# TomClabault/SYCL-ray-tracing

Hardware: AMD Instinct MI355X
Metric: Msamples/sec (W×H×spp/s) at 1080p; per-channel L∞ vs CPU ref (higher is better)
Workload: dtype f32; 1 GPU; cfg2: PBRT Dragon stand-in (1,000,002 tris) 1920x1080x64spp x8 bounces, SKY-L 2048x1024 env IS+MIS; W=1920, H=1080, spp=64, bounces=8, parallelism=1 GPU

## Files before the change

sycl-ray-tracing_amd/csrc/rt_hostsim.cpp:

```cpp
#include <omp.h>

#include <algorithm>
#include <cmath>
#include <cstdlib>
#include <cstring>
#include <vector>

#include "rt_context.h"
#include "rt_denoise.h"
#include "rt_display.h"
#include "rt_query.h"
#include "rt_wave.h"

#ifndef RT_HOSTSIM_SHORT_CAP
#define RT_HOSTSIM_SHORT_CAP 8
#endif
#ifndef RT_HOSTSIM_FAST_CAP
#define RT_HOSTSIM_FAST_CAP 32
#endif
#ifndef RT_HOSTSIM_BUDGET
#define RT_HOSTSIM_BUDGET 24
#endif

int rt_backend_create(rt_context*) { return RT_OK; }
// ... 613 lines not shown
    rtk::heap_order(k, id, m, ok, oi);
    for (int i = 0; i < m; i++) order_emul[i] = oi[i];
    struct QE {
        int id;
        float t;
        bool operator>(const QE& o) const { return t > o.t; }
    };
    std::priority_queue<QE, std::vector<QE>, std::greater<QE>> q;
    for (int i = 0; i < m; i++) q.emplace(QE{i, keys[i]});
    for (int i = 0; i < m; i++) {
        order_std[i] = q.top().id;
        q.pop();
    }
    return 0;
}

#ifndef RT_BUILD_SRC
#define RT_BUILD_SRC "unknown"
#endif
#ifndef RT_BUILD_DEFS
#define RT_BUILD_DEFS ""
#endif
extern "C" const char* rt_build_id(void) { return "src=" RT_BUILD_SRC " defs=" RT_BUILD_DEFS " (hostsim)"; }
```

sycl-ray-tracing_amd/csrc/rt_probe.hip:

```cpp
#include <hip/hip_runtime.h>

#include <algorithm>

#include "rt_backend_hip.h"
#include "rt_wave.h"
#include "rt_wave_layout.h"
#include "rt_quad.h"
#include "rt_row.h"

namespace {

#define RT_LDS_CAP_FAST 16
#define RT_SPILL_FAST RT_FAST_SPILL

template <int N, int M>
struct FastStack {
    static constexpr int CAP = N + M;
    uint32_t* r;
    float* k;
    uint32_t* gr;
    float* gk;
    __device__ __forceinline__ uint32_t rec(int i) const { return i < N ? r[i * 256] : gr[i - N]; }
    __device__ __forceinline__ float key(int i) const { return i < N ? k[i * 256] : gk[i - N]; }
    __device__ __forceinline__ void set(int i, uint32_t rv, float kv)
// ... 70 lines not shown
    const int q = (int)(threadIdx.x >> 2), sub = (int)(threadIdx.x & 3);
    rtk::QuadStack<RT_QSTACK, 64> stk{s_lds + q, (float*)s_lds + RT_QSTACK * 64 + q};
    const int stride = (int)(gridDim.x * blockDim.x) >> 2;
    for (int i = (int)((blockIdx.x * blockDim.x + threadIdx.x) >> 2); i < n; i += stride) {
        rtk::QState qs;
        int res = 1;
        if (rtk::far_origin(S, rtk::v3of(rays[2 * i])))
            res = -1;
        else if (rtk::qstate_begin<ANY>(qs, rtk::v3of(rays[2 * i]), rtk::v3of(rays[2 * i + 1]), sub, nullptr))
            do {
                res = rtk::quad_visit<ANY>(S, qs, stk, sub, nullptr);
            } while (res == 0);
        float t = -1.0f;
        int k = -1;
        const bool ok = res > 0 && (ANY || rtk::quad_closest_answer(S, qs, sub, t, k, nullptr));
        if (sub == 0) {
            if (ANY) {
                out_t[i] = ok ? (float)(qs.h.k == 1 ? 1 : 0) : -2.0f;
                out_k[i] = 0;
            } else {
                out_t[i] = ok ? t : -2.0f;
                out_k[i] = ok ? (k >= 0 ? (int)rt_asuint(S.tri4[3 * (size_t)k].w) : -1) : -2;
            }
        }
    }
}

template <bool ANY>
__global__ __launch_bounds__(256) void k_query_row(RtSceneView S, const float4_* __restrict__ rays,
                                                   float* __restrict__ out_t, int* __restrict__ out_k, int n)
{
    __shared__ uint32_t s_lds[2 * RT_RSTACK * 16];
    const int r = (int)(threadIdx.x >> 4), sub = (int)(threadIdx.x & 15);
    rtk::QuadStack<RT_RSTACK, 16> stk{s_lds + r, (float*)s_lds + RT_RSTACK * 16 + r};
    const int stride = (int)(gridDim.x * blockDim.x) >> 4;
    for (int i = (int)((blockIdx.x * blockDim.x + threadIdx.x) >> 4); i < n; i += stride) {
        rtk::QState qs;
        int res = 1;
        if (rtk::far_origin(S, rtk::v3of(rays[2 * i])))
            res = -1;
        else if (rtk::qstate_begin<ANY>(qs, rtk::v3of(rays[2 * i]), rtk::v3of(rays[2 * i + 1]), sub, nullptr))
            do {
                res = rtk::row_visit<ANY, RT_VISIT_DESCEND>(S, qs, stk, sub, nullptr);
            } while (res == 0);
        float t = -1.0f;
        int k = -1;
// ... 140 lines not shown
            case 2: hipLaunchKernelGGL((k_query<false, 1>), dim3(blocks), dim3(threads), 0, 0, b->view, d_rays, d_t, d_k, n, sr, sk); break;
            case 3: hipLaunchKernelGGL((k_query<true, 1>), dim3(blocks), dim3(threads), 0, 0, b->view, d_rays, d_t, d_k, n, sr, sk); break;
            case 4: hipLaunchKernelGGL((k_query_quad<false, 1>), dim3(qblocks), dim3(threads), 0, 0, b->view, d_rays, d_t, d_k, n); break;
            case 5: hipLaunchKernelGGL((k_query_quad<true, 1>), dim3(qblocks), dim3(threads), 0, 0, b->view, d_rays, d_t, d_k, n); break;
            case 6: hipLaunchKernelGGL((k_query_quad<false, 8>), dim3(qblocks), dim3(threads), 0, 0, b->view, d_rays, d_t, d_k, n); break;
            case 7: hipLaunchKernelGGL((k_query_quad<true, 8>), dim3(qblocks), dim3(threads), 0, 0, b->view, d_rays, d_t, d_k, n); break;
            case 8: hipLaunchKernelGGL((k_query_row<false>), dim3(rblocks), dim3(threads), 0, 0, b->view, d_rays, d_t, d_k, n); break;
            default: hipLaunchKernelGGL((k_query_row<true>), dim3(rblocks), dim3(threads), 0, 0, b->view, d_rays, d_t, d_k, n); break;
        }
    };
    launch();
    HIPCHK(c, hipGetLastError());
    HIPCHK(c, hipEventRecord(b->ev0, 0));
    for (int r = 0; r < reps; r++) launch();
    HIPCHK(c, hipEventRecord(b->ev1, 0));
    HIPCHK(c, hipEventSynchronize(b->ev1));
    float t = 0;
    HIPCHK(c, hipEventElapsedTime(&t, b->ev0, b->ev1));
    if (ms) *ms = t / reps;
    HIPCHK(c, hipMemcpy(out_t, d_t, (size_t)n * 4, hipMemcpyDeviceToHost));
    HIPCHK(c, hipMemcpy(out_k, d_k, (size_t)n * 4, hipMemcpyDeviceToHost));
    return RT_OK;
}
```

sycl-ray-tracing_amd/csrc/rt_quad.h:

```cpp
#pragma once

#include "rt_fast.h"

namespace rtk {

#define RT_QX1 0xB1
#define RT_QX2 0x4E
#define RT_QX3 0x1B

template <int CTRL>
__device__ __forceinline__ int qdpp(int v)
{
    return __builtin_amdgcn_mov_dpp(v, CTRL, 0xF, 0xF, true);
}
template <int CTRL>
__device__ __forceinline__ float qdppf(float v)
{
    return __int_as_float(qdpp<CTRL>(__float_as_int(v)));
}
__device__ __forceinline__ bool s_lower(int sub, int x) { return (sub ^ x) < sub; }
__device__ __forceinline__ int qor(int v)
{
    v |= qdpp<RT_QX1>(v);
    return v | qdpp<RT_QX2>(v);
// ... 30 lines not shown
#define RT_SLAB_QUAD RT_SLABS
#endif

struct QChild {
    int item;
    bool ok;
    float tn;
};
__device__ __forceinline__ QChild quad_child(const RtSceneView& S, int node, int sub, const RayB& rb, float tmax, V3 o,
                                             V3 d)
{
    float4_ a, b;
    child_record(S, node, sub, a, b);
#if RT_SLAB_QUAD
    const float4_ sl = S.bvh4s[4 * (size_t)node + sub];
    rt_pin(sl);
#endif
    rt_pin(a);
    rt_pin(b);
    const int ref = (int)rt_asuint(b.z), cnt = (int)rt_asuint(b.w);
    const float mn[3] = {a.x, a.y, a.z}, mx[3] = {a.w, b.x, b.y};
    QChild c;
    float tf;
    c.ok = cnt >= 0 && box_hit2(mn, mx, rb, tmax, c.tn, tf) && c.tn <= tmax;
#if RT_SLAB_QUAD
    c.ok = c.ok && slab_ok(sl, o, d, c.tn, tf);
#else
    (void)o, (void)d;
#endif
    c.item = cnt > 0 ? leaf_item(ref, cnt) : ref;
    return c;
}

template <bool MARK>
__device__ __forceinline__ float quad_tri(const RtSceneView& S, int item, int sub, V3 o, V3 d, int& k, int& leaf,
                                          int& prim)
{
    const int v = ~item;
    const int first = v >> 2, cnt = (v & 3) + 1;
    float tv = __builtin_inff();
    k = -1;
    leaf = -1;
    prim = 0x7fffffff;
    if (sub < cnt) {
        const float4_* p = S.bvh_tri4 + 3 * (first + sub);
        const float4_ a = p[0], e1 = p[1], e2 = p[2];
        rt_pin(a);
        rt_pin(e1);
        rt_pin(e2);
// ... 96 lines not shown
    q.h.tie = false;
    q.h.ovf = false;
    if (rt_isnan(d.x) || rt_isnan(d.y) || rt_isnan(d.z) || rt_isnan(o.x) || rt_isnan(o.y) || rt_isnan(o.z)) {
        q.h.t = -1.0f;
        return false;
    }
    q.rb = rayb_setup(o, d);
    q.sp = 0;
    q.cur = 0;
    return true;
}

#ifndef RT_VISIT_DESCEND
#define RT_VISIT_DESCEND 2
#endif
#define RT_BRUTE_SCENE (-1)
#define RT_BRUTE_OFF 0
#define RT_BRUTE_ON 1
template <int BRUTE>
__device__ __forceinline__ bool scene_brute(const RtSceneView& S)
{
    return BRUTE == RT_BRUTE_SCENE ? S.brute != 0 : BRUTE == RT_BRUTE_ON;
}
template <bool ANY, int DESC = RT_VISIT_DESCEND, bool PAIR = true, int BRUTE = RT_BRUTE_SCENE, class QSTK>
__device__ __forceinline__ int quad_visit(const RtSceneView& S, QState& q, QSTK& stk, int sub, Stats* st)
{
    FastHit& h = q.h;
    const bool brute = scene_brute<BRUTE>(S);
#pragma unroll 1
    for (int dd = 0; dd < DESC && q.cur >= 0; dd++) {
        if (ANY) {
            constexpr int NW = PAIR ? 2 : 1;
            int nd[NW];
            nd[0] = q.cur;
            int m = 1;
#pragma unroll
            for (int j = 1; j < NW; j++) {
                nd[j] = -1;
                if (m == j && q.sp > 0) {
                    const int t = (int)stk.rec(q.sp - 1);
                    if (t >= 0) {
                        nd[j] = t;
                        q.sp--;
                        m++;
                    }
                }
            }
            if (st && sub == 0) st->c[RT_STAT_ANY_VOL] += 4 * m;
            float4_ r0[NW], r1[NW];
#if RT_SLAB_QUAD
            float4_ sl[NW];
#endif
#pragma unroll
            for (int j = 0; j < NW; j++) {
                r0[j] = r1[j] = float4_{0.0f, 0.0f, 0.0f, 0.0f};
#if RT_SLAB_QUAD
                sl[j] = float4_{0.0f, 0.0f, -__builtin_inff(), __builtin_inff()};
                if (j < m) sl[j] = S.bvh4s[4 * (size_t)nd[j] + sub];
#endif
                if (j < m) child_record(S, nd[j], sub, r0[j], r1[j]);
            }
#pragma unroll
            for (int j = 0; j < NW; j++) {
                rt_pin(r0[j]);
                rt_pin(r1[j]);
#if RT_SLAB_QUAD
                rt_pin(sl[j]);
#endif
            }
            int base = 0, first = 0;
            bool any_first = false;
#pragma unroll
            for (int j = 0; j < NW; j++) {
                const int ref = (int)rt_asuint(r1[j].z), cnt = (int)rt_asuint(r1[j].w);
                const float mn[3] = {r0[j].x, r0[j].y, r0[j].z}, mx[3] = {r0[j].w, r1[j].x, r1[j].y};
                float tn, tf;
#if RT_SLAB_QUAD
                const bool ok = j < m && cnt >= 0 && box_hit2(mn, mx, q.rb, __builtin_inff(), tn, tf) &&
                                slab_ok(sl[j], q.o, q.d, tn, tf);
#else
                const bool ok = j < m && cnt >= 0 && box_hit2(mn, mx, q.rb, __builtin_inff(), tn, tf);
#endif
                const int item = cnt > 0 ? leaf_item(ref, cnt) : ref;
                const int o = ok ? 1 : 0;
                const int o1 = qdpp<RT_QX1>(o), o2 = qdpp<RT_QX2>(o), o3 = qdpp<RT_QX3>(o);
                const int pre = base + (s_lower(sub, 1) ? o1 : 0) + (s_lower(sub, 2) ? o2 : 0) + (s_lower(sub, 3) ? o3 : 0);
                if (ok && pre > 0) {
                    if (q.sp + pre - 1 < QSTK::CAP) stk.set_rec(q.sp + pre - 1, (uint32_t)item);
                }
                if (ok && pre == 0) {
                    first = item;
                    any_first = true;
                }
                base += o + o1 + o2 + o3;
            }
            const int nv = base;
            if (q.sp + nv - 1 > QSTK::CAP) return -1;
            if (nv > 0) {
                q.sp += nv - 1;
                q.cur = qor(any_first ? first : 0);
                continue;
            }
            q.cur = 0x7ffffffe;
            break;
        }
        if (st && sub == 0) st->c[RT_STAT_VOL] += 4;
        const float tmax = h.t + h.t * RT_T2_WINDOW;
        const QChild c = quad_child(S, q.cur, sub, q.rb, tmax, q.o, q.d);
        const float key = c.ok ? c.tn : __builtin_inff();
        const float k1 = qdppf<RT_QX1>(key), k2 = qdppf<RT_QX2>(key), k3 = qdppf<RT_QX3>(key);
        const int s1 = sub ^ 1, s2 = sub ^ 2, s3 = sub ^ 3;
        const int rank = (k1 < key || (k1 == key && s1 < sub) ? 1 : 0) + (k2 < key || (k2 == key && s2 < sub) ? 1 : 0) +
                         (k3 < key || (k3 == key && s3 < sub) ? 1 : 0);
        const int nv = qsum(c.ok ? 1 : 0);
        if (q.sp + nv - 1 > QSTK::CAP) return -1;
        if (c.ok && rank > 0) stk.set(q.sp + nv - 1 - rank, (uint32_t)c.item, key);
        if (nv > 0) {
            q.sp += nv - 1;
            q.cur = qor(c.ok && rank == 0 ? c.item : 0);
            continue;
        }
        q.cur = 0x7ffffffe;
        break;
    }
    if (q.cur >= 0 && q.cur != 0x7ffffffe) return 0;
    if (q.cur < 0) {
        if (st && sub == 0) st->c[ANY ? RT_STAT_ANY_TRI : RT_STAT_TRI] += ((~q.cur) & 3) + 1;
        int k, leaf, prim;
        const float tv = quad_tri<!ANY>(S, q.cur, sub, q.o, q.d, k, leaf, prim);
        if (ANY) {
            const int hitb = tv < __builtin_inff() ? 1 : 0;
            if (brute) {
                if (qor(hitb)) {
                    h.k = 1;
                    return 1;
                }
            } else if (int hm = qor(hitb << sub)) {
                const int l1 = qdpp<RT_QX1>(leaf), l2 = qdpp<RT_QX2>(leaf), l3 = qdpp<RT_QX3>(leaf);
                const ChainRay cr = quad_chain_ray(q.o, q.d, sub);
                int checked = -1;
#pragma unroll 1
                while (hm) {
                    const int x = (__ffs(hm) - 1) ^ sub;
                    hm &= hm - 1;
                    const int lj = x == 0 ? leaf : x == 1 ? l1 : x == 2 ? l2 : l3;
                    if (lj == checked) continue;
                    if (quad_chain_ok(S, cr, lj, false, 0.0f, sub, st)) {
                        h.k = 1;
// ... 21 lines not shown
                h.leaf = wl;
                h.prim = wp;
                h.tie = mixed;
            } else if (m1 == h.t && m1 < __builtin_inff()) {
                h.t2 = __builtin_fminf(h.t2, m2);
                if (brute) {
                    h.tie = true;
                    if (wp < h.prim) h.k = wk, h.leaf = wl, h.prim = wp;
                } else if (!mixed && wl == h.leaf) {
                    if (wk < h.k) h.k = wk, h.prim = wp;
                } else {
                    h.tie = true;
                }
            } else {
                h.t2 = __builtin_fminf(h.t2, m1);
            }
        }
    }
    if (ANY) {
        if (q.sp == 0) return 1;
        q.cur = (int)stk.rec(--q.sp);
        return 0;
    }
    const float tmax = h.t + h.t * RT_T2_WINDOW;
    int nxt = 0x7fffffff;
    while (q.sp > 0) {
        --q.sp;
        const float kk = stk.key(q.sp);
        const int rr = (int)stk.rec(q.sp);
        rt_pin(rr);
        if (kk <= tmax) {
            nxt = rr;
            break;
        }
    }
    q.cur = nxt;
    return nxt == 0x7fffffff ? 1 : 0;
}

template <int BRUTE = RT_BRUTE_SCENE>
__device__ __forceinline__ bool quad_closest_answer(const RtSceneView& S, const QState& q, int sub, float& t_out,
                                                    int& k_out, Stats* st)
{
    const FastHit& h = q.h;
    if (h.k < 0) {
        t_out = -1.0f;
        k_out = -1;
        return true;
    }
    if (RT_FUZZ_CHECK && (h.leaf & RT_FZ_BIT)) return false;
    if (scene_brute<BRUTE>(S)) {
        t_out = h.t;
        k_out = h.k;
        return true;
    }
    if (h.tie) return false;
    const float t2 = __builtin_fminf(h.t2, h.t + h.t * RT_T2_WINDOW);
    if (!quad_chain_ok(S, q.o, q.d, h.leaf, true, t2, sub, st)) return false;
    t_out = h.t;
    k_out = h.k;
// ... 18 lines not shown
```

sycl-ray-tracing_amd/csrc/rt_render.hip:

```cpp
#include <hip/hip_runtime.h>

#include "rt_backend_hip.h"
#include "rt_wave.h"
#include "rt_wave_kernels.h"
#include "rt_quad.h"
#include "rt_row.h"
#include "rt_octet.h"

namespace {

#if RT_DEBUG_FB
__device__ unsigned long long rt_dbg_fb[8];
#define RT_DBG(i) atomicAdd(&rt_dbg_fb[i], 1ull)
#else
#define RT_DBG(i) ((void)0)
#endif
__device__ __forceinline__ int lane_id() { return __lane_id(); }

template <int N>
struct LdsStack {
    static constexpr int CAP = N;
    uint32_t* r;
    float* k;
    __device__ __forceinline__ uint32_t rec(int i) const { return r[i * 256]; }
// ... 415 lines not shown
};

#if RT_DRAIN_STRONG_FENCE
#define RT_DRAIN_FENCE()                                       \
    do {                                                       \
        __builtin_amdgcn_fence(__ATOMIC_SEQ_CST, "workgroup"); \
        __builtin_amdgcn_s_waitcnt(0);                         \
        __builtin_amdgcn_wave_barrier();                       \
    } while (0)
#else
#define RT_DRAIN_FENCE()                                       \
    do {                                                       \
        __builtin_amdgcn_fence(__ATOMIC_ACQ_REL, "wavefront"); \
        __builtin_amdgcn_wave_barrier();                       \
    } while (0)
#endif

template <bool ANY, bool STATS, bool PAIR, int G, int BRUTE, class QSTK>
__device__ __forceinline__ void trace_stream(const rtk::WaveView& W, const RtSceneView& S, QSTK& stk, const int* s_pre,
                                             int first, int total, int wg, int wn, int32_t* fbn, rtk::RayRec* fbl,
                                             rtk::Stats* ps, const QPrefetch& pf)
{
    static_assert(G == 4 || G == 16, "quads or rows");
    constexpr unsigned long long ALL_IDLE = G == 4 ? 0x1111111111111111ull : 0x0001000100010001ull;
    constexpr int REFILL = G == 4 ? RT_TRACE_REFILL : 1;
    const int lane = lane_id(), qd = lane / G;
    int sub = lane & (G - 1);
    int cursor = 0;
    bool exhausted = wg * 16 >= total;
    bool active = false;
    uint32_t target = 0;
    rtk::QState q;
    if (!exhausted) queue_prefetch(W, s_pre, pf, first, cursor, wg, wn, total);
    auto finish = [&](int res, int gs) {
        if (W.r_heavy && sub == 0 && q.calls >= W.heavy_calls) W.r_heavy[target >> 3] = 1;
        if (STATS && W.iterq && sub == 0 && W.iter < RT_MAX_TIMED_ITERS) {
            int32_t* q2 = W.iterq + 2 * RT_MAX_TIMED_ITERS + 4 * W.iter;
            atomicMax(q2 + (ANY ? 1 : 0), q.calls);
            if (q.calls > 8) atomicAdd(q2 + 2, 1);
        }
        float t = 0.0f;
        int k = 0;
        int why = res < 0 ? 3 : 0;
        if (res > 0 && !ANY && !rtk::quad_closest_answer<BRUTE>(S, q, sub & 3, t, k, gs == 4 || sub == 0 ? ps : nullptr)) {
            res = -1;
            why = q.h.tie ? 1 : 2;
        }
        if (STATS && W.wlog && sub == 0 && q.calls >= W.wlog_min)
            walk_log(W, q.o, q.d, target, q.calls, res <= 0 ? -2.0f : ANY ? (float)(q.h.k == 1) : t, res <= 0 ? why : k,
                     gs == 4 ? 0 : 1);
        if (sub == 0) {
            if (res > 0) {
                if (ANY)
                    rtk::finish_any(W, target, q.h.k == 1);
                else
                    rtk::finish_closest(W, target, q.o, q.d, t, k);
            } else {
                fbl[atomicAdd(fbn, 1)] = rtk::RayRec{rtk::f4(q.o, rt_asfloat(target >> 3)),
                                                     rtk::f4(q.d, rt_asfloat(target & 7u))};
                RT_DBG(ANY ? 2 : 0);
                RT_DBG(why == 3 ? 3 : why == 1 ? 4 : 5);
                if (gs == 16) RT_DBG(6);
                atomicAdd(&W.r_park[target >> 3], 1);
                if (STATS && W.iterq && W.iter < RT_MAX_TIMED_ITERS)
                    atomicAdd(W.iterq + 2 * RT_MAX_TIMED_ITERS + 4 * W.iter + 3, 1);
            }
        }
    };
    for (;;) {
        const unsigned long long bidle = __ballot(!active && sub == 0);
        if (!exhausted && (__popcll(bidle) >= REFILL || bidle == ALL_IDLE)) {
            if (!active) {
                const int j = cursor + __popcll(bidle & ((1ull << (qd * G)) - 1ull));
                const int idx = (wg + (j >> 4) * wn) * 16 + (j & 15);
                if (idx < total) {
                    const int slot = j - cursor;
                    __builtin_amdgcn_s_waitcnt(0x0F70);
                    rtk::RayRec r;
                    r.o = pf.buf[2 * slot];
                    r.d = pf.buf[2 * slot + 1];
                    const int kind = pf.kind[slot];
                    target = (rt_asuint(r.o.w) << 3) | (uint32_t)kind;
                    if (forced_fallback(W, r.o, r.d)) {
                        if (sub == 0) {
                            r.d.w = rt_asfloat(target & 7u);
                            fbl[atomicAdd(fbn, 1)] = r;
                            atomicAdd(&W.r_park[target >> 3], 1);
                        }
                    } else if (rtk::qstate_begin<ANY>(q, rtk::v3of(r.o), rtk::v3of(r.d), sub, ps)) {
                        active = true;
                        q.calls = 0;
                    } else if (sub == 0) {
                        if (ANY)
                            rtk::finish_any(W, target, false);
                        else
                            rtk::finish_closest(W, target, q.o, q.d, -1.0f, -1);
                    }
                }
            }
            cursor += __popcll(bidle);
            exhausted = (wg + (cursor >> 4) * wn) * 16 >= total;
            __builtin_amdgcn_fence(__ATOMIC_ACQ_REL, "wavefront");
            __builtin_amdgcn_wave_barrier();
            if (!exhausted) queue_prefetch(W, s_pre, pf, first, cursor, wg, wn, total);
            if (STATS && lane == 0) ps->c[RT_STAT_REFILLS]++;
        }
        const unsigned long long bact = __ballot(active && sub == 0);
        if (!bact) {
            if (exhausted) break;
            continue;
        }
        if (G == 4 && W.drain_rows > 0 && exhausted && __popcll(bact) <= W.drain_rows) break;
        if (STATS) {
            if (active && sub == 0) ps->c[exhausted ? RT_STAT_DRAIN_VISITS : RT_STAT_QUAD_VISITS]++;
            if (lane == 0) ps->c[exhausted ? RT_STAT_DRAIN_SLOTS : RT_STAT_WAVE_SLOTS] += 64 / G;
        }
        if (active) {
            int res;
            if constexpr (G == 4)
                res = rtk::quad_visit<ANY, RT_VISIT_DESCEND, PAIR, BRUTE>(S, q, stk, sub, ps);
            else
                res = rtk::row_visit<ANY, RT_VISIT_DESCEND, BRUTE>(S, q, stk, sub, ps);
            q.calls += G == 4 ? 1 : 2;
            if (res != 0) {
                active = false;
                finish(res, G);
            }
        }
    }
    if constexpr (G == 4) {
        const unsigned long long bact = __ballot(active && sub == 0);
        if (!bact) return;
        const int row = lane >> 4;
        unsigned long long m = bact;
        for (int i = 0; i < row; i++) m &= m - 1ull;
// ... 9 lines not shown
        for (int i = 0; i < 3; i++) q.rb.inv[i] = pf(q.rb.inv[i]), q.rb.oi[i] = pf(q.rb.oi[i]);
        q.h.t = pf(q.h.t), q.h.t2 = pf(q.h.t2), q.h.k = pi(q.h.k), q.h.leaf = pi(q.h.leaf);
        if (BRUTE != RT_BRUTE_OFF) q.h.prim = pi(q.h.prim);
        q.h.tie = pi(q.h.tie ? 1 : 0) != 0;
        q.sp = pi(q.sp), q.cur = pi(q.cur), q.calls = pi(q.calls);
        target = (uint32_t)pi((int)target);
        sub = lane & 15;
        const int wq = (int)(threadIdx.x >> 6) * 16;
        uint32_t* qr = stk.r - (threadIdx.x >> 2) + wq;
        float* qk = stk.k - (threadIdx.x >> 2) + wq;
        const int sq = src >> 2;
        uint32_t r0 = 0, r1 = 0;
        float k0 = 0.0f, k1 = 0.0f;
        if (ract && sub < q.sp) r0 = qr[sub * 64 + sq], k0 = qk[sub * 64 + sq];
        if (ract && sub + 16 < q.sp) r1 = qr[(sub + 16) * 64 + sq], k1 = qk[(sub + 16) * 64 + sq];
        RT_DRAIN_FENCE();
        RowInQuadStack rs{qr + 4 * row, qk + 4 * row};
        if (ract && sub < q.sp) rs.set(sub, r0, k0);
        if (ract && sub + 16 < q.sp) rs.set(sub + 16, r1, k1);
        RT_DRAIN_FENCE();
        active = ract;
#if RT_DRAIN_RESTART == 1
        q.sp = 0;
        if (q.cur != 0x7fffffff) q.cur = 0;
#elif RT_DRAIN_RESTART == 2
        if (ract) rtk::qstate_begin<ANY>(q, q.o, q.d, sub, nullptr);
#elif RT_DRAIN_RESTART == 3
        q.rb = rtk::rayb_setup(q.o, q.d);
#elif RT_DRAIN_RESTART == 4
        q.h.t = __builtin_inff(), q.h.t2 = __builtin_inff(), q.h.k = ANY ? 0 : -1, q.h.leaf = -1;
        q.h.prim = 0x7fffffff, q.h.tie = false, q.h.ovf = false;
        q.sp = 0;
        if (q.cur != 0x7fffffff) q.cur = 0;
#endif
        while (__any(active)) {
            if (STATS) {
                if (active && sub == 0) ps->c[RT_STAT_DRAIN_VISITS]++;
                if (lane == 0) ps->c[RT_STAT_DRAIN_SLOTS] += 4;
            }
            if (active) {
                const int res = rtk::row_visit<ANY, RT_VISIT_DESCEND, BRUTE>(S, q, rs, sub, ps);
                q.calls += 2;
                if (res != 0) {
                    active = false;
                    finish(res, 16);
                }
            }
        }
    }
}

template <bool STATS, bool PAIR = true, int G = 4, int BRUTE = RT_BRUTE_SCENE>
__global__ __launch_bounds__(256) __attribute__((amdgpu_waves_per_eu(RT_TRACE_OCC, 8))) void k_trace(rtk::WaveView W, int par, unsigned long long* stats)
{
    __shared__ uint32_t s_lds[RT_LDS_WORDS * 256];
    __shared__ int s_pre[RT_NSEG + 1];
// ... 352 lines not shown
```

sycl-ray-tracing_amd/csrc/rt_row.h:

```cpp
#pragma once

#include "rt_quad.h"

namespace rtk {

#ifndef RT_SLAB_ROW
#define RT_SLAB_ROW RT_SLABS
#endif

#define RT_DPP_ROW_MIRROR 0x140
#define RT_DPP_ROW_HALF_MIRROR 0x141
#define RT_DPP_ROW_ROR(k) (0x120 + (k))

template <int CTRL>
__device__ __forceinline__ int rdpp(int v)
{
    return __builtin_amdgcn_mov_dpp(v, CTRL, 0xF, 0xF, true);
}
template <int CTRL>
__device__ __forceinline__ float rdppf(float v)
{
    return __int_as_float(rdpp<CTRL>(__float_as_int(v)));
}
__device__ __forceinline__ int row_or(int v)
// ... 18 lines not shown
    return __builtin_fminf(v, rdppf<RT_DPP_ROW_MIRROR>(v));
}
template <int K>
__device__ __forceinline__ int row_rank_from(float key, int sub)
{
    const float o = rdppf<RT_DPP_ROW_ROR(K)>(key);
    const int os = rdpp<RT_DPP_ROW_ROR(K)>(sub);
    const int c = (o < key || (o == key && os < sub)) ? 1 : 0;
    if constexpr (K < 15)
        return c + row_rank_from<K + 1>(key, sub);
    else
        return c;
}
__device__ __forceinline__ int row_rank(float key, int sub) { return row_rank_from<1>(key, sub); }

__device__ __forceinline__ unsigned row_bits(unsigned long long b) { return (unsigned)(b >> (__lane_id() & 48)) & 0xFFFFu; }

template <bool ANY, int DESC, int BRUTE = RT_BRUTE_SCENE, class RSTK>
__device__ __forceinline__ int row_visit(const RtSceneView& S, QState& q, RSTK& stk, int sub, Stats* st)
{
    FastHit& h = q.h;
    const bool brute = scene_brute<BRUTE>(S);
#pragma unroll 1
    for (int dd = 0; dd < DESC && q.cur >= 0; dd++) {
        const float4_* p = (const float4_*)(S.bvh16 + (size_t)q.cur * RT_BVH16_W + sub);
        const float4_ a = p[0], b = p[1];
#if RT_SLAB_ROW
        const float4_ sl = S.bvh16s[(size_t)q.cur * RT_BVH16_W + sub];
        rt_pin(sl);
#endif
        rt_pin(a);
        rt_pin(b);
        const int ref = (int)rt_asuint(b.z), cnt = (int)rt_asuint(b.w);
        const float mn[3] = {a.x, a.y, a.z}, mx[3] = {a.w, b.x, b.y};
        const float tmax = ANY ? __builtin_inff() : h.t + h.t * RT_T2_WINDOW;
        float tn, tf;
#if RT_SLAB_ROW
        const bool ok = cnt >= 0 && box_hit2(mn, mx, q.rb, tmax, tn, tf) && (ANY || tn <= tmax) && slab_ok(sl, q.o, q.d, tn, tf);
#else
        const bool ok = cnt >= 0 && box_hit2(mn, mx, q.rb, tmax, tn, tf) && (ANY || tn <= tmax);
#endif
        const int item = cnt > 0 ? leaf_item(ref, cnt) : ref;
        const unsigned m = row_bits(__ballot(ok));
        const int nv = __popc(m);
        if (st) {
            const int nb = __popc(row_bits(__ballot(cnt >= 0)));
            if (sub == 0) st->c[ANY ? RT_STAT_ANY_VOL : RT_STAT_VOL] += nb;
        }
        if (q.sp + nv - 1 > RSTK::CAP) return -1;
        int first;
        if (ANY) {
            const int pre = __popc(m & ((1u << sub) - 1u));
            if (ok && pre > 0) stk.set_rec(q.sp + pre - 1, (uint32_t)item);
            first = ok && pre == 0;
        } else {
            const float key = ok ? __builtin_fminf(tn, 3.0e38f) : __builtin_inff();
            const int rank = row_rank(key, sub);
            if (ok && rank > 0) stk.set(q.sp + nv - 1 - rank, (uint32_t)item, key);
            first = ok && rank == 0;
        }
        if (nv > 0) {
            q.sp += nv - 1;
            q.cur = row_or(first ? item : 0);
            continue;
        }
        q.cur = 0x7ffffffe;
        break;
    }
    if (q.cur >= 0 && q.cur != 0x7ffffffe) return 0;
    if (q.cur < 0) {
        int l0 = q.cur, l1 = 0, l2 = 0, l3 = 0, nl = 1;
        const float tw = h.t + h.t * RT_T2_WINDOW;
#pragma unroll
        for (int g = 1; g < 4; g++) {
            if (nl != g || q.sp == 0) break;
            const int t = (int)stk.rec(q.sp - 1);
            const float tk = ANY ? 0.0f : stk.key(q.sp - 1);
            if (!ANY) rt_pin(tk);
            if (t >= 0 || (!ANY && !(tk <= tw))) break;
            q.sp--;
            nl++;
            (g == 1 ? l1 : g == 2 ? l2 : l3) = t;
        }
        if (st && sub == 0) {
            int nt = ((~l0) & 3) + 1;
            if (nl > 1) nt += ((~l1) & 3) + 1;
            if (nl > 2) nt += ((~l2) & 3) + 1;
            if (nl > 3) nt += ((~l3) & 3) + 1;
            st->c[ANY ? RT_STAT_ANY_TRI : RT_STAT_TRI] += nt;
        }
        const int g = sub >> 2;
        const int mine_leaf = g == 0 ? l0 : g == 1 ? l1 : g == 2 ? l2 : l3;
// ... 36 lines not shown
                h.leaf = wl;
                h.prim = wp;
                h.tie = mixed;
            } else if (m1 == h.t && m1 < __builtin_inff()) {
                h.t2 = __builtin_fminf(h.t2, m2);
                if (brute) {
                    h.tie = true;
                    if (wp < h.prim) h.k = wk, h.leaf = wl, h.prim = wp;
                } else if (!mixed && wl == h.leaf) {
                    if (wk < h.k) h.k = wk, h.prim = wp;
                } else {
                    h.tie = true;
                }
            } else {
                h.t2 = __builtin_fminf(h.t2, m1);
            }
        }
    }
    if (ANY) {
        if (q.sp == 0) return 1;
        q.cur = (int)stk.rec(--q.sp);
        return 0;
    }
    const float tmax = h.t + h.t * RT_T2_WINDOW;
    int nxt = 0x7fffffff;
    while (q.sp > 0) {
        --q.sp;
        const float kk = stk.key(q.sp);
        const int rr = (int)stk.rec(q.sp);
        rt_pin(rr);
        if (kk <= tmax) {
            nxt = rr;
            break;
        }
    }
    q.cur = nxt;
    return nxt == 0x7fffffff ? 1 : 0;
}

}
```

sycl-ray-tracing_amd/rt_amd/_capi.py:

```python
from __future__ import annotations

import ctypes
import os

PKG_DIR = os.path.dirname(os.path.dirname(os.path.abspath(__file__)))
LIB_DIR = os.path.join(PKG_DIR, "lib")
PRODUCT = os.environ.get("RT_HIP_LIB") or os.path.join(LIB_DIR, "librt_hip.so")
HOSTSIM = os.environ.get("RT_HOSTSIM_LIB") or os.path.join(LIB_DIR, "librt_hostsim.so")

EXPORTS = [
    "rt_create", "rt_destroy", "rt_last_error", "rt_version", "rt_build_id", "rt_set_scene", "rt_build_bvh",
    "rt_set_bvh_preorder", "rt_bvh_dump", "rt_bvh_info", "rt_set_env", "rt_set_camera", "rt_render",
    "rt_render_device", "rt_render_pixels", "rt_intersect", "rt_set_stats", "rt_get_stats", "rt_last_kernel_ms",
    "rt_mesh_load", "rt_mesh_counts", "rt_mesh_copy", "rt_mesh_free", "rt_camera_preset", "rt_env_luminance_cdf",
    "rt_octree_dump", "rt_read_hdr", "rt_write_png", "rt_image_to_rgba8",
    "rt_set_intersect_mode", "rt_create_multi", "rt_device_count", "rt_set_materials", "rt_render_variants",
    "rt_create_multi_loopback", "rt_test_create_multi_rccl", "rt_test_fail_device", "rt_test_schedule", "rt_test_walk_log",
    "rt_test_walk_log_read", "rt_test_obj_parallel_min", "rt_device_env_search",
    "rt_camera_rays", "rt_render_features", "rt_render_features_device", "rt_denoise_default_params", "rt_denoise",
    "rt_denoise_device",
    "rt_query", "rt_query_device", "rt_query_last_exact",
    "rt_progress_begin", "rt_progress_advance", "rt_progress_resolve", "rt_progress_resolve_device",
    "rt_progress_info", "rt_progress_save", "rt_progress_load", "rt_progress_end",
    "rt_display_default_params", "rt_render_linear", "rt_render_linear_device", "rt_progress_resolve_linear",
# ... 72 lines not shown
    "rt_progress_begin": (I, [P, I, I, I, I, P, I, I]),
    "rt_progress_advance": (I, [P, I, P]),
    "rt_progress_resolve": (I, [P, P]),
    "rt_progress_resolve_device": (I, [P, P, P]),
    "rt_progress_info": (I, [P, P]),
    "rt_progress_save": (L, [P, P, L]),
    "rt_progress_load": (I, [P, P, L]),
    "rt_progress_end": (None, [P]),
    "rt_display_default_params": (None, [ctypes.POINTER(DisplayParams)]),
    "rt_render_linear": (I, [P, I, I, I, I, P]),
    "rt_render_linear_device": (I, [P, I, I, I, I, P, I, I, P]),
    "rt_progress_resolve_linear": (I, [P, P]),
    "rt_progress_resolve_linear_device": (I, [P, P, P]),
    "rt_display": (I, [P, I, I, P, ctypes.POINTER(DisplayParams), P, P]),
    "rt_display_device": (I, [P, I, I, P, ctypes.POINTER(DisplayParams), P, P, P]),
    "rt_write_hdr": (I, [ctypes.c_char_p, P, I, I, I]),
    "rt_device_libm": (I, [I, I, P, P, P, I]),
    "rt_device_last_kernel_ms": (ctypes.c_double, [P]),
    "rt_device_kernel_timing": (I, [P, I, P, P]),
    "rt_device_set_lanes": (I, [P, I]),
    "rt_device_last_iterations": (I, [P]),
    "rt_device_exact_handovers": (I, [P, P, I]),
    "rt_device_queries": (I, [P, I, P, I, I, P, P, P]),
    "rt_device_denoise_pass_ms": (I, [P, I, P, I]),
    "rt_device_display_kernel_ms": (I, [P, I, I, P, P, P, P, I, P]),
    "rt_hostsim_heap_order": (I, [P, I, P, P]),
    "rt_hostsim_fast_queries": (I, [P, P, I, P, P]),
    "rt_hostsim_leaf_hits": (I, [P, P, I, P]),
}

QUERY_CLOSEST, QUERY_ANY, QUERY_EXACT = 0, 1, 0x100

STAT_NAMES = ["rays", "vol", "tri", "leaf", "mat", "env", "cdf", "heap_slow", "any_rays", "any_vol", "any_tri",
              "any_leaf", "verify", "fallback", "quad_visits", "wave_slots", "refills", "drain_slots", "drain_visits",
              "steps"]

_libs: dict = {}


class RtError(RuntimeError):
    pass


def lib(hostsim: bool = False):
    path = HOSTSIM if hostsim else PRODUCT
    if path in _libs:
        return _libs[path]
    if not os.path.exists(path):
        raise RtError(f"{path} is not built: run `make` (or __graft_entry__.build()) first")
    L_ = ctypes.CDLL(path)
    for name, (res, args) in _SIGS.items():
# ... 19 lines not shown
```

Before: 1094 Msamples/s.

## Make quad BVH visit branch-free and unify refill trigger in trace loop

Rewrites the quad traversal step with bitwise predicates and select operations in place of early returns and branches. It introduces sentinel cursor states (overflow, pop, none) and a shared pop_within helper that replaces the duplicated pop loops. The wave scheduling loop now uses a single precomputed refill threshold, which also folds the drain condition into that check. The goal is to cut divergence and scalar branch overhead in the hot traversal loop. It also adds diagnostic trip-count kernels on host and device, and the heavier predicated work may add ALU cost or change drain behaviour.

```diff
diff --git a/sycl-ray-tracing_amd/csrc/rt_hostsim.cpp b/sycl-ray-tracing_amd/csrc/rt_hostsim.cpp
--- a/sycl-ray-tracing_amd/csrc/rt_hostsim.cpp
+++ b/sycl-ray-tracing_amd/csrc/rt_hostsim.cpp
@@ -659,3 +659,86 @@
 #define RT_BUILD_DEFS ""
 #endif
 extern "C" const char* rt_build_id(void) { return "src=" RT_BUILD_SRC " defs=" RT_BUILD_DEFS " (hostsim)"; }
+
+extern "C" int rt_hostsim_trip_cases(rt_context* c, const float* rays, int n, int* out)
+{
+    if (!c || n < 0 || (n > 0 && (!rays || !out))) return RT_ERR_ARG;
+    if (!c->have_bvh) return RT_ERR_STATE;
+    const RtSceneView S = rt_host_view(c);
+#pragma omp parallel
+    {
+        rtk::IdxStack<RT_HOSTSIM_FAST_CAP> stk;
+#pragma omp for schedule(dynamic, 64)
+        for (int i = 0; i < n; i++) {
+            const float* r = rays + 6 * (size_t)i;
+            const rtk::V3 o = rtk::v3(r[0], r[1], r[2]), d = rtk::v3(r[3], r[4], r[5]);
+            int* w = out + 10 * (size_t)i;
+            for (int j = 0; j < 10; j++) w[j] = 0;
+            if (rt_isnan(o.x) || rt_isnan(o.y) || rt_isnan(o.z) || rt_isnan(d.x) || rt_isnan(d.y) || rt_isnan(d.z)) continue;
+            rtk::FastHit h;
+            h.t = h.t2 = __builtin_inff();
+            h.k = -1, h.leaf = -1, h.prim = 0x7fffffff, h.tie = false, h.ovf = false;
+            const rtk::RayB rb = rtk::rayb_setup(o, d);
+            int sp = 0, cur = 0;
+            for (;;) {
+                rtk::ItemRecs R;
+                rtk::load_item(S, cur, R);
+                if (cur >= 0) {
+                    const rtk::Bvh4R nd = rtk::node_of(R);
+                    float tn[4], kk[4];
+                    bool hit[4];
+                    int v[4], ix[4] = {0, 1, 2, 3}, nv = 0;
+                    const float tmax = h.t + h.t * RT_T2_WINDOW;
+                    rtk::box4(S, cur, nd, rb, o, d, tmax, tn, hit);
+                    for (int ch = 0; ch < 4; ch++) {
+                        const bool ok = hit[ch] && tn[ch] <= tmax;
+                        kk[ch] = ok ? tn[ch] : __builtin_inff();
+                        v[ch] = nd.cnt[ch] > 0 ? rtk::leaf_item(nd.ref[ch], nd.cnt[ch]) : nd.ref[ch];
+                        nv += ok ? 1 : 0;
+                    }
+                    rtk::sort4(kk, ix);
+                    w[nv]++;
+                    for (int j = 1; j < nv; j++)
+                        if (kk[j] == kk[j - 1]) {
+                            w[5]++;
+                            break;
+                        }
+                    if (sp + nv - 1 > RT_HOSTSIM_FAST_CAP) {
+                        w[6] = sp + nv - 1;
+                        w[8] = 1;
+                        break;
+                    }
+                    for (int j = nv - 1; j >= 1; j--) stk.set(sp++, (uint32_t)v[ix[j]], kk[j]);
+                    if (sp > w[6]) w[6] = sp;
+                    if (nv > 0) {
+                        cur = v[ix[0]];
+                        continue;
+                    }
+                } else {
+                    const int cnt = ((~cur) & 3) + 1;
+                    w[9]++;
+                    for (int j = 0; j < cnt; j++) {
+                        float t;
+                        if (rtk::tri_test_v(rtk::ld3(R.q[3 * j]), rtk::ld3(R.q[3 * j + 1]), rtk::ld3(R.q[3 * j + 2]), o, d, t))
+                            rtk::fast_take(h, t, (int)rt_asuint(R.q[3 * j].w), (int)rt_asuint(R.q[3 * j + 1].w),
+                                           (int)rt_asuint(R.q[3 * j + 2].w), S.brute != 0);
+                    }
+                }
+                const float tmax = h.t + h.t * RT_T2_WINDOW;
+                cur = 0x7fffffff;
+                while (sp > 0) {
+                    --sp;
+                    if (stk.key(sp) <= tmax) {
+                        cur = (int)stk.rec(sp);
+                        break;
+                    }
+                }
+                if (cur == 0x7fffffff) {
+                    w[7]++;
+                    break;
+                }
+            }
+        }
+    }
+    return RT_OK;
+}
diff --git a/sycl-ray-tracing_amd/csrc/rt_probe.hip b/sycl-ray-tracing_amd/csrc/rt_probe.hip
--- a/sycl-ray-tracing_amd/csrc/rt_probe.hip
+++ b/sycl-ray-tracing_amd/csrc/rt_probe.hip
@@ -116,6 +116,32 @@
                 out_t[i] = ok ? t : -2.0f;
                 out_k[i] = ok ? (k >= 0 ? (int)rt_asuint(S.tri4[3 * (size_t)k].w) : -1) : -2;
             }
+        }
+    }
+}
+
+template <bool ANY>
+__global__ __launch_bounds__(256) void k_query_quad_trips(RtSceneView S, const float4_* __restrict__ rays, int* __restrict__ out, int n)
+{
+    __shared__ uint32_t s_lds[2 * RT_QSTACK * 64];
+    const int q = (int)(threadIdx.x >> 2), sub = (int)(threadIdx.x & 3);
+    rtk::QuadStack<RT_QSTACK, 64> stk{s_lds + q, (float*)s_lds + RT_QSTACK * 64 + q};
+    const int stride = (int)(gridDim.x * blockDim.x) >> 2;
+    for (int i = (int)((blockIdx.x * blockDim.x + threadIdx.x) >> 2); i < n; i += stride) {
+        rtk::QState qs;
+        rtk::Stats st;
+        for (int j = 0; j < RT_STAT_COUNT; j++) st.c[j] = 0;
+        int calls = 0, res = 1;
+        if (!rtk::far_origin(S, rtk::v3of(rays[2 * i])) &&
+            rtk::qstate_begin<ANY>(qs, rtk::v3of(rays[2 * i]), rtk::v3of(rays[2 * i + 1]), sub, &st))
+            do {
+                res = rtk::quad_visit<ANY>(S, qs, stk, sub, &st);
+                calls++;
+            } while (res == 0);
+        if (sub == 0) {
+            out[3 * i] = calls;
+            out[3 * i + 1] = (int)st.c[ANY ? RT_STAT_ANY_VOL : RT_STAT_VOL];
+            out[3 * i + 2] = (int)st.c[ANY ? RT_STAT_ANY_TRI : RT_STAT_TRI];
         }
     }
 }
@@ -302,3 +328,27 @@
     HIPCHK(c, hipMemcpy(out_k, d_k, (size_t)n * 4, hipMemcpyDeviceToHost));
     return RT_OK;
 }
+
+extern "C" int rt_device_query_trips(rt_context* c, int any, const float* rays, int n, int* out)
+{
+    if (!c || !c->backend || n <= 0 || !rays || !out || (any != 0 && any != 1)) return RT_ERR_ARG;
+    Backend* b = rt_backend_dev0(c);
+    HIPCHK(c, hipSetDevice(b->device));
+    if (c->dirty) {
+        if (int r = rt_backend_upload(c)) return r;
+        c->dirty = false;
+    }
+    const int threads = 256, qblocks = std::min((4 * n + threads - 1) / threads, 4096);
+    DevBuf b_rays, b_out;
+    if (int r = ensure(c, b_rays, (size_t)n * 32)) return r;
+    if (int r = ensure(c, b_out, (size_t)n * 12)) return r;
+    HIPCHK(c, hipMemcpy(b_rays.p, rays, (size_t)n * 32, hipMemcpyHostToDevice));
+    if (any)
+        hipLaunchKernelGGL((k_query_quad_trips<true>), dim3(qblocks), dim3(threads), 0, 0, b->view, (const float4_*)b_rays.p, (int*)b_out.p, n);
+    else
+        hipLaunchKernelGGL((k_query_quad_trips<false>), dim3(qblocks), dim3(threads), 0, 0, b->view, (const float4_*)b_rays.p, (int*)b_out.p, n);
+    HIPCHK(c, hipGetLastError());
+    HIPCHK(c, hipDeviceSynchronize());
+    HIPCHK(c, hipMemcpy(out, b_out.p, (size_t)n * 12, hipMemcpyDeviceToHost));
+    return RT_OK;
+}
diff --git a/sycl-ray-tracing_amd/csrc/rt_quad.h b/sycl-ray-tracing_amd/csrc/rt_quad.h
--- a/sycl-ray-tracing_amd/csrc/rt_quad.h
+++ b/sycl-ray-tracing_amd/csrc/rt_quad.h
@@ -76,9 +76,10 @@
     const float mn[3] = {a.x, a.y, a.z}, mx[3] = {a.w, b.x, b.y};
     QChild c;
     float tf;
-    c.ok = cnt >= 0 && box_hit2(mn, mx, rb, tmax, c.tn, tf) && c.tn <= tmax;
-#if RT_SLAB_QUAD
-    c.ok = c.ok && slab_ok(sl, o, d, c.tn, tf);
+    const bool box = box_hit2(mn, mx, rb, tmax, c.tn, tf);
+    c.ok = (cnt >= 0) & box & (c.tn <= tmax);
+#if RT_SLAB_QUAD
+    c.ok = c.ok & slab_ok(sl, o, d, c.tn, tf);
 #else
     (void)o, (void)d;
 #endif
@@ -221,13 +222,37 @@
 {
     return BRUTE == RT_BRUTE_SCENE ? S.brute != 0 : BRUTE == RT_BRUTE_ON;
 }
+constexpr int RT_CUR_OVF = 0x7ffffffd;
+constexpr int RT_CUR_POP = 0x7ffffffe;
+constexpr int RT_CUR_NONE = 0x7fffffff;
+__device__ __forceinline__ bool cur_inner(int cur) { return (unsigned)cur < (unsigned)RT_CUR_OVF; }
+
+template <class STK>
+__device__ __forceinline__ int pop_within(const STK& stk, int& sp, float tmax)
+{
+    int nxt = RT_CUR_NONE;
+    bool more;
+    do {
+        const bool has = sp > 0;
+        const int d = has ? sp - 1 : 0;
+        const float kk = stk.key(d);
+        const int rr = (int)stk.rec(d);
+        rt_pin(rr);
+        const bool take = has & (kk <= tmax);
+        nxt = take ? rr : nxt;
+        sp = d;
+        more = has & !take;
+    } while (more);
+    return nxt;
+}
+
 template <bool ANY, int DESC = RT_VISIT_DESCEND, bool PAIR = true, int BRUTE = RT_BRUTE_SCENE, class QSTK>
 __device__ __forceinline__ int quad_visit(const RtSceneView& S, QState& q, QSTK& stk, int sub, Stats* st)
 {
     FastHit& h = q.h;
     const bool brute = scene_brute<BRUTE>(S);
 #pragma unroll 1
-    for (int dd = 0; dd < DESC && q.cur >= 0; dd++) {
+    for (int dd = 0; dd < DESC && cur_inner(q.cur); dd++) {
         if (ANY) {
             constexpr int NW = PAIR ? 2 : 1;
             int nd[NW];
@@ -235,15 +260,11 @@
             int m = 1;
 #pragma unroll
             for (int j = 1; j < NW; j++) {
-                nd[j] = -1;
-                if (m == j && q.sp > 0) {
-                    const int t = (int)stk.rec(q.sp - 1);
-                    if (t >= 0) {
-                        nd[j] = t;
-                        q.sp--;
-                        m++;
-                    }
-                }
+                const int t = (int)stk.rec(q.sp > 0 ? q.sp - 1 : 0);
+                const bool tk = (m == j) & (q.sp > 0) & (t >= 0);
+                nd[j] = tk ? t : -1;
+                q.sp -= tk ? 1 : 0;
+                m += tk ? 1 : 0;
             }
             if (st && sub == 0) st->c[RT_STAT_ANY_VOL] += 4 * m;
             float4_ r0[NW], r1[NW];
@@ -268,40 +289,29 @@
 #endif
             }
             int base = 0, first = 0;
-            bool any_first = false;
 #pragma unroll
             for (int j = 0; j < NW; j++) {
                 const int ref = (int)rt_asuint(r1[j].z), cnt = (int)rt_asuint(r1[j].w);
                 const float mn[3] = {r0[j].x, r0[j].y, r0[j].z}, mx[3] = {r0[j].w, r1[j].x, r1[j].y};
                 float tn, tf;
-#if RT_SLAB_QUAD
-                const bool ok = j < m && cnt >= 0 && box_hit2(mn, mx, q.rb, __builtin_inff(), tn, tf) &&
-                                slab_ok(sl[j], q.o, q.d, tn, tf);
-#else
-                const bool ok = j < m && cnt >= 0 && box_hit2(mn, mx, q.rb, __builtin_inff(), tn, tf);
+                bool ok = (j < m) & (cnt >= 0) & box_hit2(mn, mx, q.rb, __builtin_inff(), tn, tf);
+#if RT_SLAB_QUAD
+                ok = ok & slab_ok(sl[j], q.o, q.d, tn, tf);
 #endif
                 const int item = cnt > 0 ? leaf_item(ref, cnt) : ref;
                 const int o = ok ? 1 : 0;
                 const int o1 = qdpp<RT_QX1>(o), o2 = qdpp<RT_QX2>(o), o3 = qdpp<RT_QX3>(o);
                 const int pre = base + (s_lower(sub, 1) ? o1 : 0) + (s_lower(sub, 2) ? o2 : 0) + (s_lower(sub, 3) ? o3 : 0);
-                if (ok && pre > 0) {
-                    if (q.sp + pre - 1 < QSTK::CAP) stk.set_rec(q.sp + pre - 1, (uint32_t)item);
-                }
-                if (ok && pre == 0) {
-                    first = item;
-                    any_first = true;
-                }
+                if (ok & (pre > 0) & (q.sp + pre - 1 < QSTK::CAP)) stk.set_rec(q.sp + pre - 1, (uint32_t)item);
+                first |= (ok & (pre == 0)) ? item : 0;
                 base += o + o1 + o2 + o3;
             }
             const int nv = base;
-            if (q.sp + nv - 1 > QSTK::CAP) return -1;
-            if (nv > 0) {
-                q.sp += nv - 1;
-                q.cur = qor(any_first ? first : 0);
-                continue;
-            }
-            q.cur = 0x7ffffffe;
-            break;
+            const bool ovf = q.sp + nv - 1 > QSTK::CAP;
+            const int nxt = qor(first);
+            q.sp += ((nv > 0) & !ovf) ? nv - 1 : 0;
+            q.cur = ovf ? RT_CUR_OVF : nv > 0 ? nxt : RT_CUR_POP;
+            continue;
         }
         if (st && sub == 0) st->c[RT_STAT_VOL] += 4;
         const float tmax = h.t + h.t * RT_T2_WINDOW;
@@ -312,17 +322,14 @@
         const int rank = (k1 < key || (k1 == key && s1 < sub) ? 1 : 0) + (k2 < key || (k2 == key && s2 < sub) ? 1 : 0) +
                          (k3 < key || (k3 == key && s3 < sub) ? 1 : 0);
         const int nv = qsum(c.ok ? 1 : 0);
-        if (q.sp + nv - 1 > QSTK::CAP) return -1;
-        if (c.ok && rank > 0) stk.set(q.sp + nv - 1 - rank, (uint32_t)c.item, key);
-        if (nv > 0) {
-            q.sp += nv - 1;
-            q.cur = qor(c.ok && rank == 0 ? c.item : 0);
-            continue;
-        }
-        q.cur = 0x7ffffffe;
-        break;
-    }
-    if (q.cur >= 0 && q.cur != 0x7ffffffe) return 0;
+        const bool ovf = q.sp + nv - 1 > QSTK::CAP;
+        if (c.ok & (rank > 0) & !ovf) stk.set(q.sp + nv - 1 - rank, (uint32_t)c.item, key);
+        const int nxt = qor((c.ok & (rank == 0)) ? c.item : 0);
+        q.sp += ((nv > 0) & !ovf) ? nv - 1 : 0;
+        q.cur = ovf ? RT_CUR_OVF : nv > 0 ? nxt : RT_CUR_POP;
+    }
+    if (cur_inner(q.cur)) return 0;
+    if (q.cur == RT_CUR_OVF) return -1;
     if (q.cur < 0) {
         if (st && sub == 0) st->c[ANY ? RT_STAT_ANY_TRI : RT_STAT_TRI] += ((~q.cur) & 3) + 1;
         int k, leaf, prim;
@@ -390,20 +397,8 @@
         q.cur = (int)stk.rec(--q.sp);
         return 0;
     }
-    const float tmax = h.t + h.t * RT_T2_WINDOW;
-    int nxt = 0x7fffffff;
-    while (q.sp > 0) {
-        --q.sp;
-        const float kk = stk.key(q.sp);
-        const int rr = (int)stk.rec(q.sp);
-        rt_pin(rr);
-        if (kk <= tmax) {
-            nxt = rr;
-            break;
-        }
-    }
-    q.cur = nxt;
-    return nxt == 0x7fffffff ? 1 : 0;
+    q.cur = pop_within(stk, q.sp, h.t + h.t * RT_T2_WINDOW);
+    return q.cur == RT_CUR_NONE ? 1 : 0;
 }
 
 template <int BRUTE = RT_BRUTE_SCENE>
diff --git a/sycl-ray-tracing_amd/csrc/rt_render.hip b/sycl-ray-tracing_amd/csrc/rt_render.hip
--- a/sycl-ray-tracing_amd/csrc/rt_render.hip
+++ b/sycl-ray-tracing_amd/csrc/rt_render.hip
@@ -461,7 +461,6 @@
                                              rtk::Stats* ps, const QPrefetch& pf)
 {
     static_assert(G == 4 || G == 16, "quads or rows");
-    constexpr unsigned long long ALL_IDLE = G == 4 ? 0x1111111111111111ull : 0x0001000100010001ull;
     constexpr int REFILL = G == 4 ? RT_TRACE_REFILL : 1;
     const int lane = lane_id(), qd = lane / G;
     int sub = lane & (G - 1);
@@ -506,50 +505,57 @@
             }
         }
     };
+    constexpr int NGROUPS = 64 / G;
+    static_assert(REFILL <= NGROUPS, "all groups idle triggers a refill");
+    const int trig_done = NGROUPS - (G == 4 && W.drain_rows > 0 ? min(W.drain_rows, NGROUPS) : 0);
+    int trig = exhausted ? trig_done : REFILL;
     for (;;) {
         const unsigned long long bidle = __ballot(!active && sub == 0);
-        if (!exhausted && (__popcll(bidle) >= REFILL || bidle == ALL_IDLE)) {
-            if (!active) {
-                const int j = cursor + __popcll(bidle & ((1ull << (qd * G)) - 1ull));
-                const int idx = (wg + (j >> 4) * wn) * 16 + (j & 15);
-                if (idx < total) {
-                    const int slot = j - cursor;
-                    __builtin_amdgcn_s_waitcnt(0x0F70);
-                    rtk::RayRec r;
-                    r.o = pf.buf[2 * slot];
-                    r.d = pf.buf[2 * slot + 1];
-                    const int kind = pf.kind[slot];
-                    target = (rt_asuint(r.o.w) << 3) | (uint32_t)kind;
-                    if (forced_fallback(W, r.o, r.d)) {
-                        if (sub == 0) {
-                            r.d.w = rt_asfloat(target & 7u);
-                            fbl[atomicAdd(fbn, 1)] = r;
-                            atomicAdd(&W.r_park[target >> 3], 1);
+        if (__popcll(bidle) >= trig) {
+            if (!exhausted) {
+                if (!active) {
+                    const int j = cursor + __popcll(bidle & ((1ull << (qd * G)) - 1ull));
+                    const int idx = (wg + (j >> 4) * wn) * 16 + (j & 15);
+                    if (idx < total) {
+                        const int slot = j - cursor;
+                        __builtin_amdgcn_s_waitcnt(0x0F70);
+                        rtk::RayRec r;
+                        r.o = pf.buf[2 * slot];
+                        r.d = pf.buf[2 * slot + 1];
+                        const int kind = pf.kind[slot];
+                        target = (rt_asuint(r.o.w) << 3) | (uint32_t)kind;
+                        if (forced_fallback(W, r.o, r.d)) {
+                            if (sub == 0) {
+                                r.d.w = rt_asfloat(target & 7u);
+                                fbl[atomicAdd(fbn, 1)] = r;
+                                atomicAdd(&W.r_park[target >> 3], 1);
+                            }
+                        } else if (rtk::qstate_begin<ANY>(q, rtk::v3of(r.o), rtk::v3of(r.d), sub, ps)) {
+                            active = true;
+                            q.calls = 0;
+                        } else if (sub == 0) {
+                            if (ANY)
+                                rtk::finish_any(W, target, false);
+                            else
+                                rtk::finish_closest(W, target, q.o, q.d, -1.0f, -1);
                         }
-                    } else if (rtk::qstate_begin<ANY>(q, rtk::v3of(r.o), rtk::v3of(r.d), sub, ps)) {
-                        active = true;
-                        q.calls = 0;
-                    } else if (sub == 0) {
-                        if (ANY)
-                            rtk::finish_any(W, target, false);
-                        else
-                            rtk::finish_closest(W, target, q.o, q.d, -1.0f, -1);
                     }
                 }
-            }
-            cursor += __popcll(bidle);
-            exhausted = (wg + (cursor >> 4) * wn) * 16 >= total;
-            __builtin_amdgcn_fence(__ATOMIC_ACQ_REL, "wavefront");
-            __builtin_amdgcn_wave_barrier();
-            if (!exhausted) queue_prefetch(W, s_pre, pf, first, cursor, wg, wn, total);
-            if (STATS && lane == 0) ps->c[RT_STAT_REFILLS]++;
-        }
-        const unsigned long long bact = __ballot(active && sub == 0);
-        if (!bact) {
-            if (exhausted) break;
-            continue;
-        }
-        if (G == 4 && W.drain_rows > 0 && exhausted && __popcll(bact) <= W.drain_rows) break;
+                cursor += __popcll(bidle);
+                exhausted = (wg + (cursor >> 4) * wn) * 16 >= total;
+                __builtin_amdgcn_fence(__ATOMIC_ACQ_REL, "wavefront");
+                __builtin_amdgcn_wave_barrier();
+                if (!exhausted) queue_prefetch(W, s_pre, pf, first, cursor, wg, wn, total);
+                if (STATS && lane == 0) ps->c[RT_STAT_REFILLS]++;
+                trig = exhausted ? trig_done : REFILL;
+            }
+            const unsigned long long bact = __ballot(active && sub == 0);
+            if (!bact) {
+                if (exhausted) break;
+                continue;
+            }
+            if (G == 4 && W.drain_rows > 0 && exhausted && __popcll(bact) <= W.drain_rows) break;
+        }
         if (STATS) {
             if (active && sub == 0) ps->c[exhausted ? RT_STAT_DRAIN_VISITS : RT_STAT_QUAD_VISITS]++;
             if (lane == 0) ps->c[exhausted ? RT_STAT_DRAIN_SLOTS : RT_STAT_WAVE_SLOTS] += 64 / G;
@@ -605,7 +611,7 @@
         active = ract;
 #if RT_DRAIN_RESTART == 1
         q.sp = 0;
-        if (q.cur != 0x7fffffff) q.cur = 0;
+        if (q.cur != rtk::RT_CUR_NONE) q.cur = 0;
 #elif RT_DRAIN_RESTART == 2
         if (ract) rtk::qstate_begin<ANY>(q, q.o, q.d, sub, nullptr);
 #elif RT_DRAIN_RESTART == 3
@@ -614,7 +620,7 @@
         q.h.t = __builtin_inff(), q.h.t2 = __builtin_inff(), q.h.k = ANY ? 0 : -1, q.h.leaf = -1;
         q.h.prim = 0x7fffffff, q.h.tie = false, q.h.ovf = false;
         q.sp = 0;
-        if (q.cur != 0x7fffffff) q.cur = 0;
+        if (q.cur != rtk::RT_CUR_NONE) q.cur = 0;
 #endif
         while (__any(active)) {
             if (STATS) {
diff --git a/sycl-ray-tracing_amd/csrc/rt_row.h b/sycl-ray-tracing_amd/csrc/rt_row.h
--- a/sycl-ray-tracing_amd/csrc/rt_row.h
+++ b/sycl-ray-tracing_amd/csrc/rt_row.h
@@ -64,7 +64,7 @@
     FastHit& h = q.h;
     const bool brute = scene_brute<BRUTE>(S);
 #pragma unroll 1
-    for (int dd = 0; dd < DESC && q.cur >= 0; dd++) {
+    for (int dd = 0; dd < DESC && cur_inner(q.cur); dd++) {
         const float4_* p = (const float4_*)(S.bvh16 + (size_t)q.cur * RT_BVH16_W + sub);
         const float4_ a = p[0], b = p[1];
 #if RT_SLAB_ROW
@@ -106,10 +106,10 @@
             q.cur = row_or(first ? item : 0);
             continue;
         }
-        q.cur = 0x7ffffffe;
+        q.cur = RT_CUR_POP;
         break;
     }
-    if (q.cur >= 0 && q.cur != 0x7ffffffe) return 0;
+    if (cur_inner(q.cur)) return 0;
     if (q.cur < 0) {
         int l0 = q.cur, l1 = 0, l2 = 0, l3 = 0, nl = 1;
         const float tw = h.t + h.t * RT_T2_WINDOW;
@@ -192,20 +192,8 @@
         q.cur = (int)stk.rec(--q.sp);
         return 0;
     }
-    const float tmax = h.t + h.t * RT_T2_WINDOW;
-    int nxt = 0x7fffffff;
-    while (q.sp > 0) {
-        --q.sp;
-        const float kk = stk.key(q.sp);
-        const int rr = (int)stk.rec(q.sp);
-        rt_pin(rr);
-        if (kk <= tmax) {
-            nxt = rr;
-            break;
-        }
-    }
-    q.cur = nxt;
-    return nxt == 0x7fffffff ? 1 : 0;
+    q.cur = pop_within(stk, q.sp, h.t + h.t * RT_T2_WINDOW);
+    return q.cur == RT_CUR_NONE ? 1 : 0;
 }
 
 }
diff --git a/sycl-ray-tracing_amd/rt_amd/_capi.py b/sycl-ray-tracing_amd/rt_amd/_capi.py
--- a/sycl-ray-tracing_amd/rt_amd/_capi.py
+++ b/sycl-ray-tracing_amd/rt_amd/_capi.py
@@ -118,11 +118,13 @@
     "rt_device_last_iterations": (I, [P]),
     "rt_device_exact_handovers": (I, [P, P, I]),
     "rt_device_queries": (I, [P, I, P, I, I, P, P, P]),
+    "rt_device_query_trips": (I, [P, I, P, I, P]),
     "rt_device_denoise_pass_ms": (I, [P, I, P, I]),
     "rt_device_display_kernel_ms": (I, [P, I, I, P, P, P, P, I, P]),
     "rt_hostsim_heap_order": (I, [P, I, P, P]),
     "rt_hostsim_fast_queries": (I, [P, P, I, P, P]),
     "rt_hostsim_leaf_hits": (I, [P, P, I, P]),
+    "rt_hostsim_trip_cases": (I, [P, P, I, P]),
 }
 
 QUERY_CLOSEST, QUERY_ANY, QUERY_EXACT = 0, 1, 0x100
```

Result: faster. 1113 Msamples/s (median of 6 runs) (+1.7%).
